# pierlj/ken-burns-effect

Hardware: AMD Instinct MI355X
Metric: novel_view_frames_per_sec_1024x1024 (higher is better)
Workload: dtype f32; 1 GPU; 1024x1024 KBE path, 1137109 pts (inpaint cloud), frame=shift+scatter+fill+u8+crop/resize; delivery=pinned_host, scatter_route=fused, frames_per_rank=1589, lanes=2, device_only_lanes=4, warmup_frames=3178, passes=1, handoff=sdma, ranks_seen=1

## Files before the change

### ken-burns-effect_amd/csrc/kbe_frame.hip

```cpp
#include <stdlib.h>
#include <string.h>

#include "kbe_cloud.h"
#include "kbe_handoff.h"
#include "kbe_tiles.h"

using namespace kbe;

namespace {

__global__ void k_scratch_init(uint32_t* zkeys, uint32_t* zkeys_b, size_t hw, int* tile_count, int n_tiles, int* hole_count)
{
    const size_t stride = (size_t) gridDim.x * blockDim.x, gtid = (size_t) blockIdx.x * blockDim.x + threadIdx.x;
    for (size_t i = gtid; i < hw; i += stride) { zkeys[i] = KBE_ZKEY_EMPTY; if (zkeys_b) zkeys_b[i] = KBE_ZKEY_EMPTY; }
    for (size_t i = gtid; i < (size_t) n_tiles; i += stride) { tile_count[i * CNT_STRIDE] = 0; tile_count[i * CNT_STRIDE + 1] = 0; }
    if (gtid < (size_t) HOLE_COUNT_INTS) hole_count[gtid] = 0;
}

__global__ void k_scratch_init_sets(char* base, size_t stride, size_t zkeys, size_t zkeys_b, size_t hw, size_t tile_count, int n_tiles, size_t hole_count)
{
    char* const set = base + (size_t) blockIdx.y * stride;
    uint32_t* const za = (uint32_t*) (set + zkeys), * const zb = (uint32_t*) (set + zkeys_b);
    const size_t step = (size_t) gridDim.x * blockDim.x, gtid = (size_t) blockIdx.x * blockDim.x + threadIdx.x;
    for (size_t i = gtid; i < hw; i += step) { za[i] = KBE_ZKEY_EMPTY; zb[i] = KBE_ZKEY_EMPTY; }
// ... 850 lines not shown
{
    KBE_REQUIRE(n_frames >= 0 && focals && shifts && stage && host_out && frame_size_ok(W, H) && batch >= -64 && (!packed || cloud_focal > 0.0),
                "kbe_render_video: bad arguments");
    KBE_REQUIRE((crop_w == 0 && crop_h == 0) || (crop_w > 0 && crop_h > 0 && crop_w <= W && crop_h <= H), "kbe_render_video: bad crop");
    KBE_REQUIRE(lanes >= 1 && lanes <= KBE_MAX_LANES && (lanes == 1 || lane_streams), "kbe_render_video: bad lanes");
    KBE_REQUIRE(near_depth >= 0.0 && near_depth < 1.0e30, "kbe_render_video: near_depth is a depth (0: unknown)");
    KBE_REQUIRE(scratch && ((uintptr_t) scratch & 15) == 0 && N >= 0 && (packed || (N <= (1 << 30) && (N == 0 || (points && image && depth)))),
                "kbe_render_video: bad scratch or cloud");
    const hipStream_t cs = (hipStream_t) stream;
    const size_t sb = (scratch_set_bytes(W, H, N) + 255) & ~(size_t) 255;
    const bool crop = crop_w > 0;
    const int wide_group = ((flags >> 5) & 15) + 1;
    const int group = batch <= 0 ? (wide_group > 1 ? wide_group : ((flags >> 1) & 3) + 1) : 1;
    KBE_REQUIRE(group <= (packed ? KBE_FRAME_JOBS : KBE_FILL_JOBS), "kbe_render_video: more frames per launch than the route's launches take");
    KBE_REQUIRE(!packed || N <= KBE_FUSED_MAX_POINTS, "kbe_render_video: the packed cloud's route takes up to 2^28 points (more: the plain cloud's route)");
    hipStream_t ls[KBE_MAX_LANES];
    for (int l = 0; l < lanes; l++) ls[l] = l == 0 ? cs : (hipStream_t) lane_streams[l];
    const StageLayout layout = stage_layout(W, H, lanes, batch, KBE_FRAME_JOBS);
    VideoHandoff handoff;
    if (int rc0 = handoff.open(HandoffIn{ stage, layout, host_out, batch, flags, lanes, ls, copy_stream ? (hipStream_t) copy_stream : cs })) return rc0;
    int rect[4] = { 0, 0, W - 1, H - 1 };
    if (crop) {
        const int x0 = (int) floor(W / 2.0 - (crop_w - 1) * 0.5) - 1, y0 = (int) floor(H / 2.0 - (crop_h - 1) * 0.5) - 1;
        rect[0] = x0 > 0 ? x0 : 0; rect[1] = y0 > 0 ? y0 : 0;
        rect[2] = x0 + crop_w + 2 < W - 1 ? x0 + crop_w + 2 : W - 1;
        rect[3] = y0 + crop_h + 2 < H - 1 ? y0 + crop_h + 2 : H - 1;
    }
    if (packed) {
        const Scratch sc0 = carve(scratch, W, H);
        hipLaunchKernelGGL(k_zero_counters, dim3(16, group * lanes), dim3(256), 0, cs, sc0.hole_count, sb, group * lanes, sc0.tile_count,
                           2 * align16(4 * (size_t) sc0.tiles_x * sc0.tiles_y * CNT_STRIDE) / sizeof(int));
        if (int rc0 = launched("kbe_render_video/counters")) return rc0;
    }
    const VideoPlan plan = plan_video(VideoPlanIn{ n_frames, lanes, group, batch, handoff.dest, layout.fin, (flags & KBE_VIDEO_FAST_RAMP) != 0, (flags & KBE_VIDEO_EVEN_GROUPS) != 0,
                                                   packed != nullptr, !(flags & KBE_VIDEO_NO_AHEAD) },
                                      [&](int n, int n_next) { return fused_can_place_ahead(N, W, H, n, n_next); });

    const int in_flight = plan.single ? lanes : lanes * group;
    const int fill_flags = in_flight >= KBE_FILL_BY_COUNT_MIN_LANES ? (KBE_STAGE_FILL_BY_COUNT | ((flags & KBE_VIDEO_FILL_DIST) ? KBE_STAGE_FILL_DIST : 0)) : 0;
    const int build = (flags & KBE_VIDEO_FUSED_LEAN) ? 1 : ((flags & KBE_VIDEO_FUSED_ROOMY) ? 2 : 0);
    const FillRect fill_rect = fill_rect_of(rect, W, H);
    auto fused_target_of = [&](const PlanFrame& f, uint8_t* frame, int turn) {
        return fused_target((char*) scratch + (size_t) f.set * sb, W, H, focals[f.frame], baseline, shifts + 3 * (size_t) f.frame, f.turn & 1, frame, turn);
    };
    auto render = [&](const PlanLaunch& a) {
        const hipStream_t s = ls[a.lane];
        const PlanFrame* const fr = &plan.frames[a.first];
        uint8_t* outs[KBE_FRAME_JOBS];
        uint8_t* raws[KBE_FRAME_JOBS];
        for (int j = 0; j < a.count; j++) {
            outs[j] = handoff.slot(fr[j]);
            raws[j] = crop ? stage + layout.raw(a.lane, j) : outs[j];
        }
        int rc = KBE_OK;
        if (!packed) {
            FrameJob jobs[KBE_FILL_JOBS];
            for (int j = 0; j < a.count; j++)
                jobs[j] = FrameJob{ focals[fr[j].frame], shifts + 3 * (size_t) fr[j].frame, (char*) scratch + (size_t) fr[j].set * sb, raws[j], nullptr, nullptr, nullptr, nullptr,
                                    fr[j].zbuf == PLAN_ZBUF_A ? KBE_STAGE_ZBUF_A : (fr[j].zbuf == PLAN_ZBUF_B ? KBE_STAGE_ZBUF_B : 0) };
            rc = render_jobs(points, image, depth, N, W, H, baseline, a.count, jobs, KBE_STAGE_PROJECT | KBE_STAGE_TILES | KBE_STAGE_FILL | fill_flags, crop ? rect : nullptr, raster_w, raster_n, s);
        } else if (plan.single) {
            const FusedTarget t = fused_target_of(fr[0], raws[0], -1);
            rc = render_fused(s, packed, N, cloud_focal, 1, &t, false, 0, nullptr, KBE_STAGE_TILES | KBE_STAGE_FILL | fill_flags, build, fill_rect, 0.0, "kbe_render_video");
        } else {
            FusedTarget ft[KBE_FRAME_JOBS], nt[KBE_FRAME_JOBS];
            for (int j = 0; j < a.count; j++) ft[j] = fused_target_of(fr[j], raws[j], fr[j].turn);
            const int n_next = a.next >= 0 ? plan.launches[a.next].count : 0;
            const PlanFrame* const next = n_next ? &plan.frames[plan.launches[a.next].first] : nullptr;
            for (int j = 0; j < n_next; j++) nt[j] = fused_target_of(next[j], nullptr, next[j].turn);
            rc = render_fused(s, packed, N, cloud_focal, a.count, ft, a.placed, n_next, nt, KBE_STAGE_TILES | KBE_STAGE_FILL | fill_flags, build, fill_rect, near_depth,
                              "kbe_render_video");
        }
        for (int j0 = 0; j0 < a.count && rc == KBE_OK && crop; j0 += KBE_FILL_JOBS)
            rc = crop_resize_group(a.count - j0 < KBE_FILL_JOBS ? a.count - j0 : KBE_FILL_JOBS, raws + j0, W, H, crop_w, crop_h, outs + j0, s);
        return rc;
    };

    int rc = handoff.start(plan);
    for (int u = 0; u < (int) plan.units.size() && rc == KBE_OK; u++) {
        const PlanUnit& un = plan.units[u];
        handoff.before(u, un);
        for (int a = un.launch0; a < un.launch1 && rc == KBE_OK; a++) rc = render(plan.launches[a]);
        if (rc == KBE_OK) rc = handoff.after(u, un, plan);
    }
    return handoff.finish(rc, plan);
}

}
```

### ken-burns-effect_amd/csrc/kbe_hip.hip

```cpp
#include <hip/hip_runtime.h>
#include <math.h>
#include <stdio.h>
#include <string.h>

#include "kbe.h"
#include "kbe_device.h"
#include "kbe_fill.h"
#include "kbe_host.h"

#pragma clang fp contract(off)

using namespace kbe;

thread_local char kbe::g_err[256] = "";

namespace {

__global__ void k_fill_u32(uint32_t* p, size_t n, uint32_t v)
{
    const size_t stride = (size_t) gridDim.x * blockDim.x;
    for (size_t i = (size_t) blockIdx.x * blockDim.x + threadIdx.x; i < n; i += stride) p[i] = v;
}

__global__ void k_zkeys_decode(const uint32_t* keys, size_t n, float* zee)
{
    const size_t stride = (size_t) gridDim.x * blockDim.x;
    for (size_t i = (size_t) blockIdx.x * blockDim.x + threadIdx.x; i < n; i += stride) zee[i] = zkey_decode(keys[i]);
}

__global__ void k_selftest_err(const float* __restrict__ z, size_t n, Camera cam, float* __restrict__ fast, float* __restrict__ exact)
{
    const size_t stride = (size_t) gridDim.x * blockDim.x;
    for (size_t i = (size_t) blockIdx.x * blockDim.x + threadIdx.x; i < n; i += stride) {
        fast[i] = project_err_fast(cam, z[i]);
        exact[i] = project_err(cam, z[i]);
    }
}

__global__ void k_selftest_division(const float* __restrict__ num, const float* __restrict__ den, size_t n, float* __restrict__ fast, float* __restrict__ ieee)
{
    const size_t stride = (size_t) gridDim.x * blockDim.x;
// ... 199 lines not shown

__device__ __forceinline__ void resize_coeff(int d, double scale, int src_n, bool horizontal, int& s0, int& s1, int& c0, int& c1)
{
    float f = (float) ((d + 0.5) * scale - 0.5);
    int s = (int) floorf(f);
    f -= (float) s;
    if (horizontal) {
        if (s < 0) { f = 0.f; s = 0; }
        if (s >= src_n - 1) { f = 0.f; s = src_n - 1; }
    }
    s0 = min(max(s, 0), src_n - 1);
    s1 = min(max(s + 1, 0), src_n - 1);
    c0 = cv_round((1.f - f) * 2048.f);
    c1 = cv_round(f * 2048.f);
}

__device__ __forceinline__ uint32_t mul_u24_v(uint32_t a, uint32_t b) { uint32_t r; asm("v_mul_u32_u24 %0, %1, %2" : "=v"(r) : "v"(a), "v"(b)); return r; }
__device__ __forceinline__ uint32_t mad_u24_v(uint32_t a, uint32_t b, uint32_t c) { uint32_t r; asm("v_mad_u32_u24 %0, %1, %2, %3" : "=v"(r) : "v"(a), "v"(b), "v"(c)); return r; }
__device__ __forceinline__ uint32_t mul_u24_s(uint32_t a, uint32_t b) { uint32_t r; asm("v_mul_u32_u24 %0, %1, %2" : "=v"(r) : "s"(a), "v"(b)); return r; }
__device__ __forceinline__ uint32_t mul_hi_u24_s(uint32_t a, uint32_t b) { uint32_t r; asm("v_mul_hi_u32_u24 %0, %1, %2" : "=v"(r) : "s"(a), "v"(b)); return r; }
__device__ __forceinline__ uint32_t mad_u24_s(uint32_t a, uint32_t b, uint32_t c) { uint32_t r; asm("v_mad_u32_u24 %0, %1, %2, %3" : "=v"(r) : "s"(a), "v"(b), "v"(c)); return r; }

#ifndef KBE_CROP_TH
#define KBE_CROP_TH 16
#endif
constexpr int CR_TW = 64, CR_TH = KBE_CROP_TH, CR_THREADS = 256, CR_WAVES = CR_THREADS / 64;
constexpr int CR_ROWS_PER_WAVE = CR_TH / CR_WAVES;
constexpr int CR_PROWS = CR_TH + 2, CR_PCOLS = CR_TW + 2;
constexpr int CR_PBYTES = CR_PCOLS * 3, CR_PSTRIDE = (CR_PBYTES + 3) / 4 + 1;
constexpr int CR_RROWS = CR_PROWS + 1, CR_RDW = ((CR_PCOLS + 1) * 3 + 3 + 3) / 4 + 1;
constexpr int CR_STAGE = (CR_RROWS + CR_WAVES - 1) / CR_WAVES;
static_assert(CR_TH % CR_WAVES == 0 && CR_RDW <= 64 && CR_PBYTES <= CR_THREADS && CR_TW + CR_TH <= CR_THREADS && CR_PROWS + 1 <= CR_THREADS, "crop tile geometry");

__device__ __forceinline__ void crop_resize_body(const uint8_t* __restrict__ img, int W, int H, int cw, int ch_, double scale_x, double scale_y, uint8_t* __restrict__ out)
{
    __shared__ uint32_t s_raw[CR_RROWS][CR_RDW];
    __shared__ uint32_t s_patch[CR_PROWS][CR_PSTRIDE];
    __shared__ __attribute__((aligned(16))) uint32_t s_out[CR_TH][CR_TW * 3 / 4];
    __shared__ int s_cx[4][CR_TW], s_cy[4][CR_TH];
    __shared__ int s_ro[CR_PROWS + 1];
    const int tid = threadIdx.x;
    const int bx = blockIdx.x * CR_TW, by = blockIdx.y * CR_TH;
    const float cx = (float) W / 2.0f - (float) (cw - 1) * 0.5f, cy = (float) H / 2.0f - (float) (ch_ - 1) * 0.5f;
    const int ipx = (int) floorf(cx), ipy = (int) floorf(cy);
    const float fa = cx - (float) ipx, fb = cy - (float) ipy;
    const int a11 = cv_round((1.f - fa) * (1.f - fb) * 65536.f), a12 = cv_round(fa * (1.f - fb) * 65536.f);
    const int a21 = cv_round((1.f - fa) * fb * 65536.f), a22 = cv_round(fa * fb * 65536.f);
    const bool whole = (a12 | a21 | a22) == 0;
    if (tid < CR_TW + CR_TH) {
        const bool col = tid < CR_TW;
        const int k = col ? tid : tid - CR_TW;
        int s0, s1, c0, c1;
        if (col) resize_coeff(min(bx + k, W - 1), scale_x, cw, true, s0, s1, c0, c1);
        else resize_coeff(min(by + k, H - 1), scale_y, ch_, false, s0, s1, c0, c1);
        int* t = col ? &s_cx[0][k] : &s_cy[0][k];
        const int stride = col ? CR_TW : CR_TH;
        t[0] = s0; t[stride] = s1; t[2 * stride] = c0; t[3 * stride] = c1;
    }
    __syncthreads();
    const int px_lo = s_cx[0][0], px_hi = s_cx[1][CR_TW - 1], py_lo = s_cy[0][0], py_hi = s_cy[1][CR_TH - 1];
    const int n_pc3 = (px_hi - px_lo + 1) * 3, n_pr = py_hi - py_lo + 1;
    const int rx0 = min(max(ipx + px_lo, 0), W - 1), rx1 = min(max(ipx + px_hi + 1, 0), W - 1);
    const int ry0 = min(max(ipy + py_lo, 0), H - 1), ry1 = min(max(ipy + py_hi + 1, 0), H - 1);
    const int n_rows = ry1 - ry0 + 1;
    const size_t frame_bytes = (size_t) W * H * 3;
    const int wv = __builtin_amdgcn_readfirstlane(tid >> 6), ln = tid & 63;
    uint32_t stage[CR_STAGE];
#pragma unroll
    for (int k = 0; k < CR_STAGE; k++) {
        const int r = wv + CR_WAVES * k;
        stage[k] = 0;
        if (r < n_rows) {
            const size_t b0 = ((size_t) (ry0 + r) * W + rx0) * 3, b1 = ((size_t) (ry0 + r) * W + rx1) * 3 + 3;
            const size_t a0 = b0 & ~(size_t) 3;
            const int n_dw = (int) ((b1 - a0 + 3) >> 2);
            const uint8_t* row = img + a0;
            if (a0 + 4 * (size_t) n_dw <= frame_bytes) {
                if (ln < n_dw) stage[k] = ((const uint32_t*) row)[ln];
            } else if (ln < n_dw) {
                for (int t = 0; t < 4; t++) if (a0 + 4 * (size_t) ln + t < frame_bytes) stage[k] |= (uint32_t) row[4 * ln + t] << (8 * t);
            }
        }
    }
#pragma unroll
    for (int k = 0; k < CR_STAGE; k++) {
        const int r = wv + CR_WAVES * k;
        if (r < CR_RROWS && ln < CR_RDW) s_raw[r][ln] = stage[k];
    }
    if (tid <= CR_PROWS) {
        const int y = min(max(ipy + py_lo + tid, 0), H - 1);
        s_ro[tid] = min(y - ry0, CR_RROWS - 1) * (int) sizeof(s_raw[0]) + (int) ((((uint32_t) y * (uint32_t) W + (uint32_t) rx0) * 3u) & 3u);
    }
    __syncthreads();
    const uint8_t* raw = (const uint8_t*) s_raw;
    uint8_t* patch = (uint8_t*) s_patch;
    if (!whole) {
        if (tid < n_pc3) {
            const int pc = tid / 3, c = tid - pc * 3;
            const int x0 = (min(max(ipx + px_lo + pc, 0), W - 1) - rx0) * 3 + c, x1 = (min(max(ipx + px_lo + pc + 1, 0), W - 1) - rx0) * 3 + c;
            int o = s_ro[0];
            int t0 = raw[o + x0], t1 = raw[o + x1];
            for (int pr = 0; pr < n_pr; pr++) {
                o = s_ro[pr + 1];
                const int u0 = raw[o + x0], u1 = raw[o + x1];
                const uint32_t t = mad_u24_s((uint32_t) a22, (uint32_t) u1, mad_u24_s((uint32_t) a21, (uint32_t) u0, mad_u24_s((uint32_t) a12, (uint32_t) t1, mad_u24_s((uint32_t) a11, (uint32_t) t0, 1u << 15))));
                patch[pr * (int) sizeof(s_patch[0]) + tid] = (uint8_t) (t >> 16);
                t0 = u0; t1 = u1;
            }
        }
        __syncthreads();
    }
    const int col = tid & (CR_TW - 1);
    const uint8_t* const src = whole ? raw : (const uint8_t*) patch;
    int sx, sx1;
    if (whole) {
        sx = (min(max(ipx + s_cx[0][col], 0), W - 1) - rx0) * 3;
        sx1 = (min(max(ipx + s_cx[1][col], 0), W - 1) - rx0) * 3;
    } else {
        sx = (s_cx[0][col] - px_lo) * 3;
        sx1 = (s_cx[1][col] - px_lo) * 3;
    }
    const int ax0 = s_cx[2][col], ax1 = s_cx[3][col];
    auto row_offset = [&](int pr) -> int {
        return whole ? s_ro[pr] : pr * (int) sizeof(s_patch[0]);
    };
    auto horizontal = [&](int pr, int (&h)[3]) {
        const int o = row_offset(pr);
#pragma unroll
        for (int c = 0; c < 3; c++) h[c] = (int) (mad_u24_v(src[o + sx1 + c], (uint32_t) ax1, mul_u24_v(src[o + sx + c], (uint32_t) ax0)) & ~15u);
    };
    int ka = -1, kb = -1;
    int ha[3] = { 0, 0, 0 }, hb[3] = { 0, 0, 0 };
    uint8_t px[CR_ROWS_PER_WAVE][3];
#pragma unroll
    for (int m = 0; m < CR_ROWS_PER_WAVE; m++) {
        const int row = wv * CR_ROWS_PER_WAVE + m;
        const int y0 = __builtin_amdgcn_readfirstlane(s_cy[0][row] - py_lo), y1 = __builtin_amdgcn_readfirstlane(s_cy[1][row] - py_lo);
        const int by0 = __builtin_amdgcn_readfirstlane(s_cy[2][row]), by1 = __builtin_amdgcn_readfirstlane(s_cy[3][row]);
        if (ka != y0) {
            if (kb == y0) {
#pragma unroll
                for (int c = 0; c < 3; c++) ha[c] = hb[c];
            } else horizontal(y0, ha);
            ka = y0;
        }
        if (y1 == y0) {
#pragma unroll
            for (int c = 0; c < 3; c++) hb[c] = ha[c];
            kb = y0;
        } else if (kb != y1) { horizontal(y1, hb); kb = y1; }
#pragma unroll
        for (int c = 0; c < 3; c++) {
            const uint32_t v = (mul_hi_u24_s((uint32_t) by0 << 12, (uint32_t) ha[c]) + mul_hi_u24_s((uint32_t) by1 << 12, (uint32_t) hb[c]) + 2u) >> 2;
            px[m][c] = (uint8_t) v;
        }
        uint8_t* so = (uint8_t*) s_out[row] + col * 3;
        so[0] = px[m][0]; so[1] = px[m][1]; so[2] = px[m][2];
    }
    __syncthreads();
    if ((W & 15) == 0 && bx + CR_TW <= W && ((uintptr_t) out & 15) == 0) {
        constexpr int Q = CR_TW * 3 / 16;
        static_assert((CR_TW * 3) % 16 == 0 && sizeof(s_out[0]) % 16 == 0, "16-byte row stores");
        for (int i = tid; i < CR_TH * Q; i += CR_THREADS) {
            const int r = i / Q, k = i - r * Q;
            if (by + r < H) ((uint4*) (out + ((size_t) (by + r) * W + bx) * 3))[k] = ((const uint4*) s_out[r])[k];
        }
    } else if ((W & 3) == 0 && bx + CR_TW <= W && ((uintptr_t) out & 3) == 0) {
        constexpr int DW = CR_TW * 3 / 4;
        for (int i = tid; i < CR_TH * DW; i += CR_THREADS) {
            const int r = i / DW, k = i - r * DW;
            if (by + r < H) ((uint32_t*) (out + ((size_t) (by + r) * W + bx) * 3))[k] = s_out[r][k];
        }
    } else {
#pragma unroll
        for (int m = 0; m < CR_ROWS_PER_WAVE; m++) {
            const int dx = bx + col, dy = by + wv * CR_ROWS_PER_WAVE + m;
            if (dx < W && dy < H) {
                const size_t o = ((size_t) dy * W + dx) * 3;
                out[o] = px[m][0]; out[o + 1] = px[m][1]; out[o + 2] = px[m][2];
            }
        }
    }
}

__global__ void __launch_bounds__(CR_THREADS) k_crop_resize_u8(const uint8_t* __restrict__ img, int W, int H, int cw, int ch_, double scale_x, double scale_y,
                                                               uint8_t* __restrict__ out)
{
    crop_resize_body(img, W, H, cw, ch_, scale_x, scale_y, out);
}

struct CropJobs { const uint8_t* img[4]; uint8_t* out[4]; };
__global__ void __launch_bounds__(CR_THREADS) k_crop_resize_u8_group(CropJobs jobs, int W, int H, int cw, int ch_, double scale_x, double scale_y)
{
    crop_resize_body(jobs.img[blockIdx.z], W, H, cw, ch_, scale_x, scale_y, jobs.out[blockIdx.z]);
}


__device__ __forceinline__ float linspace_centered(int n, int i)
{
    const float start = (float) ((-0.5 * n) + 0.5), end = (float) ((0.5 * n) - 0.5);
    if (n == 1) return start;
    const float step = (end - start) / (float) (n - 1);
    return (i < n / 2) ? start + step * (float) i : end - step * (float) (n - 1 - i);
}

__global__ void __launch_bounds__(kBlock) k_depth_to_points(const float* __restrict__ depth, const float* __restrict__ valid,
                                                            int W, int H, float inv_focal, float* __restrict__ points)
{
    const int b = blockIdx.y;
    const int HW = W * H;
    const int i = blockIdx.x * blockDim.x + threadIdx.x;
    if (i >= HW) return;
    const int y = i / W, x = i - y * W;
    float d = depth[(size_t) b * HW + i];
    if (valid) d = d * valid[(size_t) b * HW + i];
    const float u = linspace_centered(W, x) * inv_focal;
    const float v = linspace_centered(H, y) * inv_focal;
    float* P = points + (size_t) b * 3 * HW;
    P[i] = d * u;
    P[(size_t) HW + i] = d * v;
    P[(size_t) 2 * HW + i] = d;
}

__global__ void __launch_bounds__(kBlock) k_shift_points(const float* __restrict__ points, int N, Camera cam,
                                                         float* __restrict__ out)
{
    const int b = blockIdx.y;
// ... 316 lines not shown
    int rc;
    if ((rc = kbe_zkeys_clear(zkeys, (size_t) B * H * W, stream))) return rc;
    const hipError_t e = hipMemsetAsync(acc, 0, sizeof(float) * (size_t) B * (C + 1) * H * W, (hipStream_t) stream);
    if (e != hipSuccess) return fail(KBE_E_LAUNCH, "hipMemsetAsync(acc)", e);
    if ((rc = kbe_zsplat(points, B, N, W, H, focal, baseline, nullptr, zkeys, nullptr, stream))) return rc;
    if ((rc = kbe_degrid(zkeys, nullptr, B, W, H, zee, stream))) return rc;
    if ((rc = kbe_accumulate(points, data, B, N, C, zee, W, H, focal, baseline, nullptr, acc, stream))) return rc;
    return kbe_normalize(acc, B, C, W, H, render, existing, stream);
}

int kbe_fill_disocclusion(const float* input, const float* depth, int B, int C, int W, int H, float* output,
                          kbe_stream_t stream)
{
    KBE_REQUIRE(input && depth && output && B > 0 && C > 0 && W > 0 && H > 0, "kbe_fill_disocclusion: bad arguments");
    static const FillDirs dirs = make_fill_dirs();
    hipLaunchKernelGGL(k_fill, dim3(blocks_for((size_t) W * H), B), dim3(kBlock), 0, (hipStream_t) stream, input, depth, C,
                       W, H, dirs, output);
    return launched("kbe_fill_disocclusion");
}

int kbe_frame_u8(const float* render_chw, int W, int H, uint8_t* frame_hwc, kbe_stream_t stream)
{
    KBE_REQUIRE(render_chw && frame_hwc && W > 0 && H > 0, "kbe_frame_u8: bad arguments");
    hipLaunchKernelGGL(k_frame_u8, dim3(blocks_for((size_t) W * H)), dim3(kBlock), 0, (hipStream_t) stream, render_chw,
                       W * H, frame_hwc);
    return launched("kbe_frame_u8");
}

int kbe_crop_resize_u8(const uint8_t* frame_hwc, int W, int H, int crop_w, int crop_h, uint8_t* out_hwc,
                       kbe_stream_t stream)
{
    KBE_REQUIRE(frame_hwc && out_hwc && W > 0 && H > 0 && crop_w > 0 && crop_h > 0 && crop_w <= W && crop_h <= H,
                "kbe_crop_resize_u8: bad arguments");
    hipLaunchKernelGGL(k_crop_resize_u8, dim3((W + CR_TW - 1) / CR_TW, (H + CR_TH - 1) / CR_TH), dim3(CR_THREADS), 0,
                       (hipStream_t) stream, frame_hwc, W, H, crop_w, crop_h, (double) crop_w / W, (double) crop_h / H, out_hwc);
    return launched("kbe_crop_resize_u8");
}

}

namespace kbe {
int crop_resize_group(int n, const uint8_t* const* frames, int W, int H, int crop_w, int crop_h, uint8_t* const* outs, hipStream_t stream)
{
    if (n == 1) return kbe_crop_resize_u8(frames[0], W, H, crop_w, crop_h, outs[0], (kbe_stream_t) stream);
    CropJobs jobs;
    for (int k = 0; k < 4; k++) { jobs.img[k] = frames[k < n ? k : 0]; jobs.out[k] = outs[k < n ? k : 0]; }
    hipLaunchKernelGGL(k_crop_resize_u8_group, dim3((W + CR_TW - 1) / CR_TW, (H + CR_TH - 1) / CR_TH, n), dim3(CR_THREADS), 0, stream, jobs, W, H, crop_w, crop_h, (double) crop_w / W, (double) crop_h / H);
    return launched("kbe_crop_resize_u8 (group)");
}
}

extern "C" {

int kbe_depth_to_points(const float* depth, const float* valid, int B, int W, int H, double focal, float* points,
                        kbe_stream_t stream)
{
    KBE_REQUIRE(depth && points && B > 0 && W > 0 && H > 0, "kbe_depth_to_points: bad arguments");
    const float inv = (float) (1.0 / focal);
    hipLaunchKernelGGL(k_depth_to_points, dim3(blocks_for((size_t) W * H), B), dim3(kBlock), 0, (hipStream_t) stream, depth,
                       valid, W, H, inv, points);
    return launched("kbe_depth_to_points");
}

int kbe_shift_points(const float* points, int B, int N, const float* shift3, float* out, kbe_stream_t stream)
{
    KBE_REQUIRE(shift3 && B > 0 && N >= 0, "kbe_shift_points: bad arguments");
    if (N == 0) return KBE_OK;
    KBE_REQUIRE(points && out, "kbe_shift_points: points/out is NULL");
    const Camera cam = make_camera(1, 1, 1.0, 1.0, shift3);
    hipLaunchKernelGGL(k_shift_points, dim3(blocks_for(N), B), dim3(kBlock), 0, (hipStream_t) stream, points, N, cam, out);
    return launched("kbe_shift_points");
}

int kbe_spatial_filter(const float* in, int planes, int W, int H, int kind, float* out, kbe_stream_t stream)
{
    KBE_REQUIRE(in && out && planes > 0 && W > 0 && H > 0, "kbe_spatial_filter: bad arguments");
    const dim3 grid(blocks_for((size_t) W * H), planes);
    const hipStream_t s = (hipStream_t) stream;
    if (kind == 0) {
        hipLaunchKernelGGL(k_laplacian<false>, grid, dim3(kBlock), 0, s, in, (const float*) nullptr, W, H, 0.0f, out);
// ... 60 lines not shown
```

### ken-burns-effect_amd/csrc/kbe_tiles.h

```cpp
#pragma once
#include <hip/hip_runtime.h>
#include <math.h>
#include <stddef.h>
#include <stdint.h>
#include <type_traits>

#include "kbe.h"
#include "kbe_device.h"
#include "kbe_fill.h"
#include "kbe_host.h"
#include "kbe_cloud.h"

#pragma clang fp contract(off)

namespace kbe {

#ifndef KBE_TILE_W
#define KBE_TILE_W 32
#endif
#ifndef KBE_TILE_H
#define KBE_TILE_H 16
#endif
#ifndef KBE_TILE_THREADS
#define KBE_TILE_THREADS 256
#endif
#ifndef KBE_TILE_CAP
#define KBE_TILE_CAP 736
#endif
#ifndef KBE_BUCKET_FACTOR
#define KBE_BUCKET_FACTOR 12
#endif
constexpr int TW = KBE_TILE_W, TH = KBE_TILE_H;
constexpr int KW = TW + 2, KH = TH + 2;
constexpr int BW = TW + 1, BH = TH + 1;
constexpr int TILE_THREADS = KBE_TILE_THREADS;
constexpr int PIX_PER_THREAD = TW * TH / TILE_THREADS;
constexpr int REC_CAP = KBE_TILE_CAP;
constexpr int BUCKET_CAP = KBE_BUCKET_FACTOR * TW * TH;
#ifndef KBE_BUCKET_PAD
#define KBE_BUCKET_PAD 272
#endif
constexpr int BUCKET_STRIDE = BUCKET_CAP + KBE_BUCKET_PAD;
#ifndef KBE_CAND_CAP
#define KBE_CAND_CAP (2048 * 16 / KBE_CLOUD_SUB)
#endif
constexpr int CNT_STRIDE = 32;
static_assert(TW * TH % TILE_THREADS == 0 && TILE_THREADS % 64 == 0 && REC_CAP >= TILE_THREADS && TW % 32 == 0, "tile geometry");

struct Scratch {
    uint32_t* zkeys;
    uint32_t* zkeys_b;
    uint8_t* dist;
    float2* strips;
    uint8_t* dist_blocks;
    int* tile_count;
    int* hole_count;
    int4* bbox;
    uint32_t* coarse;
    int* holes;
    float* depth;
    uint32_t* mask;
    int* cand;
    float4* buckets;
    int tiles_x, tiles_y;
};

inline size_t align16(size_t v) { return (v + 15) & ~(size_t) 15; }

inline Scratch carve(void* base, int W, int H)
{
    char* p = (char*) base;
    const size_t hw = (size_t) W * H;
    Scratch s;
    s.tiles_x = (W + TW - 1) / TW;
    s.tiles_y = (H + TH - 1) / TH;
    const size_t n_tiles = (size_t) s.tiles_x * s.tiles_y;
    s.zkeys = (uint32_t*) p;      p += align16(4 * hw);
    s.tile_count = (int*) p;      p += 2 * align16(4 * n_tiles * CNT_STRIDE);
    s.hole_count = (int*) p;      p += 32;
    s.bbox = (int4*) p;           p += align16(16 * n_tiles);
    s.coarse = (uint32_t*) p;     p += align16(4 * n_tiles);
    s.holes = (int*) p;           p += align16(4 * hw);
    s.depth = (float*) p;         p += align16(4 * hw);
    s.mask = (uint32_t*) p;       p += align16(4 * (size_t) H * ((W + 31) / 32));
    s.zkeys_b = (uint32_t*) p;    p += align16(4 * hw);
    s.dist = (uint8_t*) p;        p += align16(hw);
    s.strips = (float2*) p;       p += align16(8 * 16 * (size_t) (W + H + 8));
    s.dist_blocks = (uint8_t*) p; p += align16(n_tiles * (TW / 8) * (TH / 8));
    s.cand = (int*) p;            p += 2 * align16(4 * n_tiles * KBE_CAND_CAP);
    s.buckets = (float4*) p;
    return s;
}

inline size_t scratch_bytes(int W, int H)
{
    const size_t hw = (size_t) W * H;
    const size_t n_tiles = (size_t) ((W + TW - 1) / TW) * ((H + TH - 1) / TH);
    return align16(4 * hw) + 2 * align16(4 * n_tiles * CNT_STRIDE) + 32 + align16(16 * n_tiles) + align16(4 * n_tiles) + align16(4 * hw) + align16(4 * hw) +
           align16(4 * (size_t) H * ((W + 31) / 32)) + align16(4 * hw) + align16(hw) + align16(8 * 16 * (size_t) (W + H + 8)) + align16(n_tiles * (TW / 8) * (TH / 8)) + 2 * align16(4 * n_tiles * KBE_CAND_CAP) + n_tiles * BUCKET_STRIDE * sizeof(float4);
}


size_t fused_place_bytes(int N);
inline size_t scratch_set_bytes(int W, int H, int N) { return align16(scratch_bytes(W, H)) + (N >= 0 ? 2 * align16(fused_place_bytes(N)) : 0); }
inline void* scratch_place(void* base, int W, int H) { return (char*) base + align16(scratch_bytes(W, H)); }
inline int* bank_tile_count(const Scratch& s, int bank) { return (int*) ((char*) s.tile_count + (size_t) bank * align16(4 * (size_t) s.tiles_x * s.tiles_y * CNT_STRIDE)); }
inline int* bank_cand(const Scratch& s, int bank) { return (int*) ((char*) s.cand + (size_t) bank * align16(4 * (size_t) s.tiles_x * s.tiles_y * KBE_CAND_CAP)); }
inline void* bank_place(void* place, int N, int bank) { return (char*) place + (size_t) bank * align16(fused_place_bytes(N)); }
constexpr int HOLE_COUNT_INTS = 8;

struct FillRect { int x0, y0, x1, y1; };

#ifndef KBE_FILL_BY_COUNT_MIN_LANES
#define KBE_FILL_BY_COUNT_MIN_LANES 2
#endif

constexpr int KBE_FILL_JOBS = 4;
#ifndef KBE_FRAME_JOBS_MAX
#define KBE_FRAME_JOBS_MAX 12
#endif
constexpr int KBE_FUSED_MAX_POINTS = 1 << 28;
constexpr int KBE_FRAME_JOBS = KBE_FRAME_JOBS_MAX;
struct FillTarget {
    Scratch sc;
    const int* hole_count;
    uint8_t* frame_u8;
    float* render_f32;
    int reset_scatter_scratch;
    int* next_hole_count;
};
struct FillJob {
    const int* holes; const int* hole_count; const float* depth; const uint32_t* mask; uint8_t* frame; float* render;
    uint32_t* zkeys; int* tile_count; const int4* bbox; const uint32_t* coarse; uint8_t* dist; float2* strips; uint8_t* dist_blocks;
    int reset_scatter_scratch; int* next_hole_count;
};
struct FillJobs { FillJob j[KBE_FILL_JOBS]; };
void launch_fill(hipStream_t s, int n_jobs, const FillTarget* targets, int W, int H, int stages, const FillDirs& dirs, const FillRect& rect, int n_tiles);
int crop_resize_group(int n, const uint8_t* const* frames, int W, int H, int crop_w, int crop_h, uint8_t* const* outs, hipStream_t stream);
struct FusedTarget {
    Camera cam;
    Scratch sc;
    void* place;
    int parity;
    uint8_t* frame_u8;
    float* render_f32; float* existing_f32; float* zee_f32; float* zee_pre_f32;
    int turn;
};
void launch_frames_fused(hipStream_t s, int n, const void* packed, int N, double cloud_focal, const FusedTarget* targets, bool placed = false, int n_next = 0,
                         const FusedTarget* next = nullptr, int build = 0, double near_depth = 0.0);
inline int fused_build_of_stages(int stages) { return (stages & 1024) ? 1 : ((stages & 2048) ? 2 : 0); }
bool fused_can_place_ahead(int N, int W, int H, int n, int n_next);

__device__ __forceinline__ int xcd_tile(int b, int n)
{
    const int xcd = b & 7, j = b >> 3, q = n >> 3, r = n & 7;
    return (xcd < r ? xcd * (q + 1) : r * (q + 1) + (xcd - r) * q) + j;
}
__device__ __forceinline__ int xcd_tile_rot(int b, int n, int job)
{
    if (n & 7) return xcd_tile(b, n);
    const int stride = gridDim.y >= 8 ? 1 : 8 / (int) gridDim.y;
    return (((b + job * stride) & 7) * (n >> 3)) + (b >> 3);
}

typedef float f2 __attribute__((ext_vector_type(2)));
typedef float f4 __attribute__((ext_vector_type(4)));
struct PixAcc { f2 rg, bd; float w; };

template <int CAP> struct TileLdsT {
    static constexpr int kCap = CAP;
    static constexpr int kDummy = CAP;
// ... 239 lines not shown
```

### ken-burns-effect_amd/csrc/kbe_video_plan.h

```cpp
#pragma once
#include <stddef.h>
#include <vector>

namespace kbe {

enum class VideoDest {
    HBM,
    PER_FRAME,
    GROUPS,
    RING,
};
enum { PLAN_ZBUF_ALONE = 0, PLAN_ZBUF_A = 1, PLAN_ZBUF_B = 2 };

struct StageLayout {
    size_t fb;
    int fin;
    size_t raw_per_lane, finished, ring, ctl, total;
    size_t raw(int lane, int j) const { return (raw_per_lane * lane + j) * fb; }
};
inline StageLayout stage_layout(int W, int H, int lanes, int batch, int raw_per_lane)
{
    const size_t fb = (size_t) W * H * 3, fin = batch < -2 ? -batch : 2;
    const size_t finished = (size_t) raw_per_lane * lanes * fb, ring = finished + fin * lanes * fb;
    const size_t ctl = (ring + 2 * (size_t) (batch > 0 ? batch : 0) * fb + 255) & ~(size_t) 255;
    return StageLayout{ fb, (int) fin, (size_t) raw_per_lane, finished, ring, ctl, ctl + 256 };
}

struct VideoPlanIn {
    int n_frames, lanes, group, batch;
    VideoDest dest;
    int fin;
    bool fast_ramp, even_groups;
    bool fused;
    bool ahead;
};
struct PlanFrame {
    int frame;
    int set;
    int turn;
    int zbuf;
    int slot;
};
struct PlanLaunch {
    int lane, first, count;
    bool placed;
    int next;
};
struct PlanUnit {
    int lane;
    int first, count;
    int launch0, launch1;
};
struct VideoPlan {
    bool single;
    std::vector<PlanUnit> units;
    std::vector<PlanLaunch> launches;
    std::vector<PlanFrame> frames;
};
// ... 71 lines not shown
```

Before: 17750 frames/s.

## Precompute crop-resize coefficient table once per video and specialize kernel on whole-pixel crop

```diff
diff --git a/ken-burns-effect_amd/csrc/kbe_frame.hip b/ken-burns-effect_amd/csrc/kbe_frame.hip
--- a/ken-burns-effect_amd/csrc/kbe_frame.hip
+++ b/ken-burns-effect_amd/csrc/kbe_frame.hip
@@ -906,6 +906,9 @@
                            2 * align16(4 * (size_t) sc0.tiles_x * sc0.tiles_y * CNT_STRIDE) / sizeof(int));
         if (int rc0 = launched("kbe_render_video/counters")) return rc0;
     }
+    int* const crop_table = carve(scratch, W, H).crop_table;
+    if (crop)
+        if (int rc0 = crop_table_build(W, H, crop_w, crop_h, crop_table, cs)) return rc0;
     const VideoPlan plan = plan_video(VideoPlanIn{ n_frames, lanes, group, batch, handoff.dest, layout.fin, (flags & KBE_VIDEO_FAST_RAMP) != 0, (flags & KBE_VIDEO_EVEN_GROUPS) != 0,
                                                    packed != nullptr, !(flags & KBE_VIDEO_NO_AHEAD) },
                                       [&](int n, int n_next) { return fused_can_place_ahead(N, W, H, n, n_next); });
@@ -946,7 +949,7 @@
                               "kbe_render_video");
         }
         for (int j0 = 0; j0 < a.count && rc == KBE_OK && crop; j0 += KBE_FILL_JOBS)
-            rc = crop_resize_group(a.count - j0 < KBE_FILL_JOBS ? a.count - j0 : KBE_FILL_JOBS, raws + j0, W, H, crop_w, crop_h, outs + j0, s);
+            rc = crop_resize_group(a.count - j0 < KBE_FILL_JOBS ? a.count - j0 : KBE_FILL_JOBS, raws + j0, W, H, crop_w, crop_h, outs + j0, crop_table, s);
         return rc;
     };
 
diff --git a/ken-burns-effect_amd/csrc/kbe_hip.hip b/ken-burns-effect_amd/csrc/kbe_hip.hip
--- a/ken-burns-effect_amd/csrc/kbe_hip.hip
+++ b/ken-burns-effect_amd/csrc/kbe_hip.hip
@@ -2,11 +2,16 @@
 #include <math.h>
 #include <stdio.h>
 #include <string.h>
+#include <type_traits>
+#ifdef KBE_DEBUG
+#include <assert.h>
+#endif
 
 #include "kbe.h"
 #include "kbe_device.h"
 #include "kbe_fill.h"
 #include "kbe_host.h"
+#include "kbe_video_plan.h"
 
 #pragma clang fp contract(off)
 
@@ -272,53 +277,143 @@
 constexpr int CR_STAGE = (CR_RROWS + CR_WAVES - 1) / CR_WAVES;
 static_assert(CR_TH % CR_WAVES == 0 && CR_RDW <= 64 && CR_PBYTES <= CR_THREADS && CR_TW + CR_TH <= CR_THREADS && CR_PROWS + 1 <= CR_THREADS, "crop tile geometry");
 
-__device__ __forceinline__ void crop_resize_body(const uint8_t* __restrict__ img, int W, int H, int cw, int ch_, double scale_x, double scale_y, uint8_t* __restrict__ out)
-{
-    __shared__ uint32_t s_raw[CR_RROWS][CR_RDW];
-    __shared__ uint32_t s_patch[CR_PROWS][CR_PSTRIDE];
-    __shared__ __attribute__((aligned(16))) uint32_t s_out[CR_TH][CR_TW * 3 / 4];
-    __shared__ int s_cx[4][CR_TW], s_cy[4][CR_TH];
-    __shared__ int s_ro[CR_PROWS + 1];
-    const int tid = threadIdx.x;
-    const int bx = blockIdx.x * CR_TW, by = blockIdx.y * CR_TH;
+template <class RowOffset>
+__device__ __forceinline__ void crop_resize_rows(const uint8_t* src, int sx, int sx1, int ax0, int ax1, const int4 (&cye)[CR_ROWS_PER_WAVE], int py_lo, int wv, int col,
+                                                 RowOffset row_offset, uint32_t (&s_out)[CR_TH][CR_TW * 3 / 4])
+{
+    auto horizontal = [&](int pr, int (&h)[3]) {
+        const int o = row_offset(pr);
+#pragma unroll
+        for (int c = 0; c < 3; c++) h[c] = (int) (mad_u24_v(src[o + sx1 + c], (uint32_t) ax1, mul_u24_v(src[o + sx + c], (uint32_t) ax0)) & ~15u);
+    };
+    int ka = -1, kb = -1;
+    int ha[3] = { 0, 0, 0 }, hb[3] = { 0, 0, 0 };
+#pragma unroll
+    for (int m = 0; m < CR_ROWS_PER_WAVE; m++) {
+        const int row = wv * CR_ROWS_PER_WAVE + m;
+        const int y0 = cye[m].x - py_lo, y1 = cye[m].y - py_lo;
+        const int by0 = cye[m].z, by1 = cye[m].w;
+        if (ka != y0) {
+            if (kb == y0) {
+#pragma unroll
+                for (int c = 0; c < 3; c++) ha[c] = hb[c];
+            } else horizontal(y0, ha);
+            ka = y0;
+        }
+        if (y1 == y0) {
+#pragma unroll
+            for (int c = 0; c < 3; c++) hb[c] = ha[c];
+            kb = y0;
+        } else if (kb != y1) { horizontal(y1, hb); kb = y1; }
+        uint8_t* so = (uint8_t*) s_out[row] + col * 3;
+#pragma unroll
+        for (int c = 0; c < 3; c++) {
+            const uint32_t v = (mul_hi_u24_s((uint32_t) by0 << 12, (uint32_t) ha[c]) + mul_hi_u24_s((uint32_t) by1 << 12, (uint32_t) hb[c]) + 2u) >> 2;
+            so[c] = (uint8_t) v;
+        }
+    }
+}
+
+struct CropHeader { int ipx, ipy, a11, a12, a21, a22, whole, pad; };
+static_assert(sizeof(CropHeader) == crop_table_layout(1, 1).cols && crop_table_layout(3, 1).rows == sizeof(CropHeader) + 3 * sizeof(int4), "the table's header: 8 dwords, then the columns, then the rows (kbe_video_plan.h: crop_table_layout)");
+__host__ __device__ __forceinline__ CropHeader crop_header(int W, int H, int cw, int ch_)
+{
     const float cx = (float) W / 2.0f - (float) (cw - 1) * 0.5f, cy = (float) H / 2.0f - (float) (ch_ - 1) * 0.5f;
     const int ipx = (int) floorf(cx), ipy = (int) floorf(cy);
     const float fa = cx - (float) ipx, fb = cy - (float) ipy;
-    const int a11 = cv_round((1.f - fa) * (1.f - fb) * 65536.f), a12 = cv_round(fa * (1.f - fb) * 65536.f);
-    const int a21 = cv_round((1.f - fa) * fb * 65536.f), a22 = cv_round(fa * fb * 65536.f);
-    const bool whole = (a12 | a21 | a22) == 0;
-    if (tid < CR_TW + CR_TH) {
-        const bool col = tid < CR_TW;
-        const int k = col ? tid : tid - CR_TW;
-        int s0, s1, c0, c1;
-        if (col) resize_coeff(min(bx + k, W - 1), scale_x, cw, true, s0, s1, c0, c1);
-        else resize_coeff(min(by + k, H - 1), scale_y, ch_, false, s0, s1, c0, c1);
-        int* t = col ? &s_cx[0][k] : &s_cy[0][k];
-        const int stride = col ? CR_TW : CR_TH;
-        t[0] = s0; t[stride] = s1; t[2 * stride] = c0; t[3 * stride] = c1;
-    }
-    __syncthreads();
-    const int px_lo = s_cx[0][0], px_hi = s_cx[1][CR_TW - 1], py_lo = s_cy[0][0], py_hi = s_cy[1][CR_TH - 1];
+    const int a11 = (int) rintf((1.f - fa) * (1.f - fb) * 65536.f), a12 = (int) rintf(fa * (1.f - fb) * 65536.f);
+    const int a21 = (int) rintf((1.f - fa) * fb * 65536.f), a22 = (int) rintf(fa * fb * 65536.f);
+    return CropHeader{ ipx, ipy, a11, a12, a21, a22, (a12 | a21 | a22) == 0, 0 };
+}
+
+__global__ void __launch_bounds__(kBlock) k_crop_table(int W, int H, int cw, int ch_, double scale_x, double scale_y, int* __restrict__ table)
+{
+    const int i = blockIdx.x * blockDim.x + threadIdx.x;
+    if (i == 0) *(CropHeader*) table = crop_header(W, H, cw, ch_);
+    if (i >= W + H) return;
+    int s0, s1, c0, c1;
+    if (i < W) resize_coeff(i, scale_x, cw, true, s0, s1, c0, c1);
+    else resize_coeff(i - W, scale_y, ch_, false, s0, s1, c0, c1);
+    ((int4*) (table + sizeof(CropHeader) / sizeof(int)))[i] = make_int4(s0, s1, c0, c1);
+}
+
+template <bool WHOLE, bool TABLE>
+__device__ __forceinline__ void crop_resize_body(const uint8_t* __restrict__ img, int W, int H, int cw, int ch_, double scale_x, double scale_y,
+                                                 const int* __restrict__ table, uint8_t* __restrict__ out)
+{
+    using offs_t = std::conditional_t<TABLE, uint32_t, size_t>;
+    __shared__ uint32_t s_raw[CR_RROWS][CR_RDW];
+    __shared__ __attribute__((aligned(16))) uint32_t s_out[CR_TH][CR_TW * 3 / 4];
+    const int tid = threadIdx.x;
+    const int bx = blockIdx.x * CR_TW, by = blockIdx.y * CR_TH;
+    const int wv = __builtin_amdgcn_readfirstlane(tid >> 6), ln = tid & 63;
+    const int col = tid & (CR_TW - 1);
+    auto uni = [](int v) { return __builtin_amdgcn_readfirstlane(v); };
+    CropHeader hd;
+    int4 cxe, cye[CR_ROWS_PER_WAVE];
+    int px_lo, px_hi, py_lo, py_hi;
+    if constexpr (TABLE) {
+        const CropHeader* const th = (const CropHeader*) table;
+        const int4* const cols = (const int4*) (table + sizeof(CropHeader) / sizeof(int));
+        const int4* const rows = cols + W;
+        hd.ipx = uni(th->ipx); hd.ipy = uni(th->ipy);
+        if constexpr (!WHOLE) { hd.a11 = uni(th->a11); hd.a12 = uni(th->a12); hd.a21 = uni(th->a21); hd.a22 = uni(th->a22); }
+#ifdef KBE_DEBUG
+        assert((th->whole != 0) == WHOLE);
+#endif
+        cxe = cols[min(bx + col, W - 1)];
+#pragma unroll
+        for (int m = 0; m < CR_ROWS_PER_WAVE; m++) {
+            const int4 e = rows[min(by + wv * CR_ROWS_PER_WAVE + m, H - 1)];
+            cye[m] = make_int4(uni(e.x), uni(e.y), uni(e.z), uni(e.w));
+        }
+        px_lo = uni(cols[min(bx, W - 1)].x); px_hi = uni(cols[min(bx + CR_TW - 1, W - 1)].y);
+        py_lo = uni(rows[min(by, H - 1)].x); py_hi = uni(rows[min(by + CR_TH - 1, H - 1)].y);
+    } else {
+        __shared__ int s_cx[4][CR_TW], s_cy[4][CR_TH];
+        hd = crop_header(W, H, cw, ch_);
+#ifdef KBE_DEBUG
+        assert((hd.whole != 0) == WHOLE);
+#endif
+        if (tid < CR_TW + CR_TH) {
+            const bool is_col = tid < CR_TW;
+            const int k = is_col ? tid : tid - CR_TW;
+            int s0, s1, c0, c1;
+            if (is_col) resize_coeff(min(bx + k, W - 1), scale_x, cw, true, s0, s1, c0, c1);
+            else resize_coeff(min(by + k, H - 1), scale_y, ch_, false, s0, s1, c0, c1);
+            int* t = is_col ? &s_cx[0][k] : &s_cy[0][k];
+            const int stride = is_col ? CR_TW : CR_TH;
+            t[0] = s0; t[stride] = s1; t[2 * stride] = c0; t[3 * stride] = c1;
+        }
+        __syncthreads();
+        cxe = make_int4(s_cx[0][col], s_cx[1][col], s_cx[2][col], s_cx[3][col]);
+#pragma unroll
+        for (int m = 0; m < CR_ROWS_PER_WAVE; m++) {
+            const int row = wv * CR_ROWS_PER_WAVE + m;
+            cye[m] = make_int4(uni(s_cy[0][row]), uni(s_cy[1][row]), uni(s_cy[2][row]), uni(s_cy[3][row]));
+        }
+        px_lo = uni(s_cx[0][0]); px_hi = uni(s_cx[1][CR_TW - 1]); py_lo = uni(s_cy[0][0]); py_hi = uni(s_cy[1][CR_TH - 1]);
+    }
+    const int ipx = hd.ipx, ipy = hd.ipy;
     const int n_pc3 = (px_hi - px_lo + 1) * 3, n_pr = py_hi - py_lo + 1;
     const int rx0 = min(max(ipx + px_lo, 0), W - 1), rx1 = min(max(ipx + px_hi + 1, 0), W - 1);
     const int ry0 = min(max(ipy + py_lo, 0), H - 1), ry1 = min(max(ipy + py_hi + 1, 0), H - 1);
     const int n_rows = ry1 - ry0 + 1;
-    const size_t frame_bytes = (size_t) W * H * 3;
-    const int wv = __builtin_amdgcn_readfirstlane(tid >> 6), ln = tid & 63;
+    const offs_t frame_bytes = (offs_t) W * H * 3;
     uint32_t stage[CR_STAGE];
 #pragma unroll
     for (int k = 0; k < CR_STAGE; k++) {
         const int r = wv + CR_WAVES * k;
         stage[k] = 0;
         if (r < n_rows) {
-            const size_t b0 = ((size_t) (ry0 + r) * W + rx0) * 3, b1 = ((size_t) (ry0 + r) * W + rx1) * 3 + 3;
-            const size_t a0 = b0 & ~(size_t) 3;
+            const offs_t b0 = ((offs_t) (ry0 + r) * W + rx0) * 3, b1 = ((offs_t) (ry0 + r) * W + rx1) * 3 + 3;
+            const offs_t a0 = b0 & ~(offs_t) 3;
             const int n_dw = (int) ((b1 - a0 + 3) >> 2);
             const uint8_t* row = img + a0;
-            if (a0 + 4 * (size_t) n_dw <= frame_bytes) {
+            if (a0 + 4 * (offs_t) n_dw <= frame_bytes) {
                 if (ln < n_dw) stage[k] = ((const uint32_t*) row)[ln];
             } else if (ln < n_dw) {
-                for (int t = 0; t < 4; t++) if (a0 + 4 * (size_t) ln + t < frame_bytes) stage[k] |= (uint32_t) row[4 * ln + t] << (8 * t);
+                for (int t = 0; t < 4; t++) if (a0 + 4 * (offs_t) ln + t < frame_bytes) stage[k] |= (uint32_t) row[4 * ln + t] << (8 * t);
             }
         }
     }
@@ -327,14 +422,21 @@
         const int r = wv + CR_WAVES * k;
         if (r < CR_RROWS && ln < CR_RDW) s_raw[r][ln] = stage[k];
     }
-    if (tid <= CR_PROWS) {
-        const int y = min(max(ipy + py_lo + tid, 0), H - 1);
-        s_ro[tid] = min(y - ry0, CR_RROWS - 1) * (int) sizeof(s_raw[0]) + (int) ((((uint32_t) y * (uint32_t) W + (uint32_t) rx0) * 3u) & 3u);
-    }
-    __syncthreads();
+    auto raw_row_offset = [&](int pr) -> int {
+        const int y = min(max(ipy + py_lo + pr, 0), H - 1);
+        return min(y - ry0, CR_RROWS - 1) * (int) sizeof(s_raw[0]) + (int) ((((uint32_t) y * (uint32_t) W + (uint32_t) rx0) * 3u) & 3u);
+    };
     const uint8_t* raw = (const uint8_t*) s_raw;
-    uint8_t* patch = (uint8_t*) s_patch;
-    if (!whole) {
+    if constexpr (WHOLE) {
+        __syncthreads();
+        const int sx = (min(max(ipx + cxe.x, 0), W - 1) - rx0) * 3, sx1 = (min(max(ipx + cxe.y, 0), W - 1) - rx0) * 3;
+        crop_resize_rows(raw, sx, sx1, cxe.z, cxe.w, cye, py_lo, wv, col, raw_row_offset, s_out);
+    } else {
+        __shared__ uint32_t s_patch[CR_PROWS][CR_PSTRIDE];
+        __shared__ int s_ro[CR_PROWS + 1];
+        if (tid <= CR_PROWS) s_ro[tid] = raw_row_offset(tid);
+        __syncthreads();
+        uint8_t* patch = (uint8_t*) s_patch;
         if (tid < n_pc3) {
             const int pc = tid / 3, c = tid - pc * 3;
             const int x0 = (min(max(ipx + px_lo + pc, 0), W - 1) - rx0) * 3 + c, x1 = (min(max(ipx + px_lo + pc + 1, 0), W - 1) - rx0) * 3 + c;
@@ -343,59 +445,13 @@
             for (int pr = 0; pr < n_pr; pr++) {
                 o = s_ro[pr + 1];
                 const int u0 = raw[o + x0], u1 = raw[o + x1];
-                const uint32_t t = mad_u24_s((uint32_t) a22, (uint32_t) u1, mad_u24_s((uint32_t) a21, (uint32_t) u0, mad_u24_s((uint32_t) a12, (uint32_t) t1, mad_u24_s((uint32_t) a11, (uint32_t) t0, 1u << 15))));
+                const uint32_t t = mad_u24_s((uint32_t) hd.a22, (uint32_t) u1, mad_u24_s((uint32_t) hd.a21, (uint32_t) u0, mad_u24_s((uint32_t) hd.a12, (uint32_t) t1, mad_u24_s((uint32_t) hd.a11, (uint32_t) t0, 1u << 15))));
                 patch[pr * (int) sizeof(s_patch[0]) + tid] = (uint8_t) (t >> 16);
                 t0 = u0; t1 = u1;
             }
         }
         __syncthreads();
-    }
-    const int col = tid & (CR_TW - 1);
-    const uint8_t* const src = whole ? raw : (const uint8_t*) patch;
-    int sx, sx1;
-    if (whole) {
-        sx = (min(max(ipx + s_cx[0][col], 0), W - 1) - rx0) * 3;
-        sx1 = (min(max(ipx + s_cx[1][col], 0), W - 1) - rx0) * 3;
-    } else {
-        sx = (s_cx[0][col] - px_lo) * 3;
-        sx1 = (s_cx[1][col] - px_lo) * 3;
-    }
-    const int ax0 = s_cx[2][col], ax1 = s_cx[3][col];
-    auto row_offset = [&](int pr) -> int {
-        return whole ? s_ro[pr] : pr * (int) sizeof(s_patch[0]);
-    };
-    auto horizontal = [&](int pr, int (&h)[3]) {
-        const int o = row_offset(pr);
-#pragma unroll
-        for (int c = 0; c < 3; c++) h[c] = (int) (mad_u24_v(src[o + sx1 + c], (uint32_t) ax1, mul_u24_v(src[o + sx + c], (uint32_t) ax0)) & ~15u);
-    };
-    int ka = -1, kb = -1;
-    int ha[3] = { 0, 0, 0 }, hb[3] = { 0, 0, 0 };
-    uint8_t px[CR_ROWS_PER_WAVE][3];
-#pragma unroll
-    for (int m = 0; m < CR_ROWS_PER_WAVE; m++) {
-        const int row = wv * CR_ROWS_PER_WAVE + m;
-        const int y0 = __builtin_amdgcn_readfirstlane(s_cy[0][row] - py_lo), y1 = __builtin_amdgcn_readfirstlane(s_cy[1][row] - py_lo);
-        const int by0 = __builtin_amdgcn_readfirstlane(s_cy[2][row]), by1 = __builtin_amdgcn_readfirstlane(s_cy[3][row]);
-        if (ka != y0) {
-            if (kb == y0) {
-#pragma unroll
-                for (int c = 0; c < 3; c++) ha[c] = hb[c];
-            } else horizontal(y0, ha);
-            ka = y0;
-        }
-        if (y1 == y0) {
-#pragma unroll
-            for (int c = 0; c < 3; c++) hb[c] = ha[c];
-            kb = y0;
-        } else if (kb != y1) { horizontal(y1, hb); kb = y1; }
-#pragma unroll
-        for (int c = 0; c < 3; c++) {
-            const uint32_t v = (mul_hi_u24_s((uint32_t) by0 << 12, (uint32_t) ha[c]) + mul_hi_u24_s((uint32_t) by1 << 12, (uint32_t) hb[c]) + 2u) >> 2;
-            px[m][c] = (uint8_t) v;
-        }
-        uint8_t* so = (uint8_t*) s_out[row] + col * 3;
-        so[0] = px[m][0]; so[1] = px[m][1]; so[2] = px[m][2];
+        crop_resize_rows(patch, (cxe.x - px_lo) * 3, (cxe.y - px_lo) * 3, cxe.z, cxe.w, cye, py_lo, wv, col, [](int pr) -> int { return pr * (int) sizeof(s_patch[0]); }, s_out);
     }
     __syncthreads();
     if ((W & 15) == 0 && bx + CR_TW <= W && ((uintptr_t) out & 15) == 0) {
@@ -403,36 +459,40 @@
         static_assert((CR_TW * 3) % 16 == 0 && sizeof(s_out[0]) % 16 == 0, "16-byte row stores");
         for (int i = tid; i < CR_TH * Q; i += CR_THREADS) {
             const int r = i / Q, k = i - r * Q;
-            if (by + r < H) ((uint4*) (out + ((size_t) (by + r) * W + bx) * 3))[k] = ((const uint4*) s_out[r])[k];
+            if (by + r < H) ((uint4*) (out + ((offs_t) (by + r) * W + bx) * 3))[k] = ((const uint4*) s_out[r])[k];
         }
     } else if ((W & 3) == 0 && bx + CR_TW <= W && ((uintptr_t) out & 3) == 0) {
         constexpr int DW = CR_TW * 3 / 4;
         for (int i = tid; i < CR_TH * DW; i += CR_THREADS) {
             const int r = i / DW, k = i - r * DW;
-            if (by + r < H) ((uint32_t*) (out + ((size_t) (by + r) * W + bx) * 3))[k] = s_out[r][k];
+            if (by + r < H) ((uint32_t*) (out + ((offs_t) (by + r) * W + bx) * 3))[k] = s_out[r][k];
         }
     } else {
 #pragma unroll
         for (int m = 0; m < CR_ROWS_PER_WAVE; m++) {
-            const int dx = bx + col, dy = by + wv * CR_ROWS_PER_WAVE + m;
+            const int row = wv * CR_ROWS_PER_WAVE + m;
+            const int dx = bx + col, dy = by + row;
             if (dx < W && dy < H) {
-                const size_t o = ((size_t) dy * W + dx) * 3;
-                out[o] = px[m][0]; out[o + 1] = px[m][1]; out[o + 2] = px[m][2];
+                const offs_t o = ((offs_t) dy * W + dx) * 3;
+                const uint8_t* so = (const uint8_t*) s_out[row] + col * 3;
+                out[o] = so[0]; out[o + 1] = so[1]; out[o + 2] = so[2];
             }
         }
     }
 }
 
+template <bool WHOLE>
 __global__ void __launch_bounds__(CR_THREADS) k_crop_resize_u8(const uint8_t* __restrict__ img, int W, int H, int cw, int ch_, double scale_x, double scale_y,
                                                                uint8_t* __restrict__ out)
 {
-    crop_resize_body(img, W, H, cw, ch_, scale_x, scale_y, out);
+    crop_resize_body<WHOLE, false>(img, W, H, cw, ch_, scale_x, scale_y, nullptr, out);
 }
 
 struct CropJobs { const uint8_t* img[4]; uint8_t* out[4]; };
-__global__ void __launch_bounds__(CR_THREADS) k_crop_resize_u8_group(CropJobs jobs, int W, int H, int cw, int ch_, double scale_x, double scale_y)
-{
-    crop_resize_body(jobs.img[blockIdx.z], W, H, cw, ch_, scale_x, scale_y, jobs.out[blockIdx.z]);
+template <bool WHOLE>
+__global__ void __launch_bounds__(CR_THREADS) k_crop_resize_u8_group(CropJobs jobs, int W, int H, int cw, int ch_, const int* __restrict__ table)
+{
+    crop_resize_body<WHOLE, true>(jobs.img[blockIdx.z], W, H, cw, ch_, 0.0, 0.0, table, jobs.out[blockIdx.z]);
 }
 
 
@@ -815,7 +875,8 @@
 {
     KBE_REQUIRE(frame_hwc && out_hwc && W > 0 && H > 0 && crop_w > 0 && crop_h > 0 && crop_w <= W && crop_h <= H,
                 "kbe_crop_resize_u8: bad arguments");
-    hipLaunchKernelGGL(k_crop_resize_u8, dim3((W + CR_TW - 1) / CR_TW, (H + CR_TH - 1) / CR_TH), dim3(CR_THREADS), 0,
+    const auto kernel = crop_header(W, H, crop_w, crop_h).whole ? k_crop_resize_u8<true> : k_crop_resize_u8<false>;
+    hipLaunchKernelGGL(kernel, dim3((W + CR_TW - 1) / CR_TW, (H + CR_TH - 1) / CR_TH), dim3(CR_THREADS), 0,
                        (hipStream_t) stream, frame_hwc, W, H, crop_w, crop_h, (double) crop_w / W, (double) crop_h / H, out_hwc);
     return launched("kbe_crop_resize_u8");
 }
@@ -823,12 +884,20 @@
 }
 
 namespace kbe {
-int crop_resize_group(int n, const uint8_t* const* frames, int W, int H, int crop_w, int crop_h, uint8_t* const* outs, hipStream_t stream)
-{
-    if (n == 1) return kbe_crop_resize_u8(frames[0], W, H, crop_w, crop_h, outs[0], (kbe_stream_t) stream);
+int crop_table_build(int W, int H, int crop_w, int crop_h, int* table, hipStream_t stream)
+{
+    KBE_REQUIRE(table && ((uintptr_t) table & 15) == 0 && W > 0 && H > 0 && crop_w > 0 && crop_h > 0 && crop_w <= W && crop_h <= H, "crop_table_build: bad arguments");
+    hipLaunchKernelGGL(k_crop_table, dim3(blocks_for((size_t) W + H)), dim3(kBlock), 0, stream, W, H, crop_w, crop_h, (double) crop_w / W, (double) crop_h / H, table);
+    return launched("kbe_crop_resize_u8 (table)");
+}
+
+int crop_resize_group(int n, const uint8_t* const* frames, int W, int H, int crop_w, int crop_h, uint8_t* const* outs, const int* table, hipStream_t stream)
+{
+    KBE_REQUIRE(n >= 1 && n <= 4 && table && (size_t) W * H <= (1u << 30), "crop_resize_group: bad arguments");
     CropJobs jobs;
     for (int k = 0; k < 4; k++) { jobs.img[k] = frames[k < n ? k : 0]; jobs.out[k] = outs[k < n ? k : 0]; }
-    hipLaunchKernelGGL(k_crop_resize_u8_group, dim3((W + CR_TW - 1) / CR_TW, (H + CR_TH - 1) / CR_TH, n), dim3(CR_THREADS), 0, stream, jobs, W, H, crop_w, crop_h, (double) crop_w / W, (double) crop_h / H);
+    const auto kernel = crop_header(W, H, crop_w, crop_h).whole ? k_crop_resize_u8_group<true> : k_crop_resize_u8_group<false>;
+    hipLaunchKernelGGL(kernel, dim3((W + CR_TW - 1) / CR_TW, (H + CR_TH - 1) / CR_TH, n), dim3(CR_THREADS), 0, stream, jobs, W, H, crop_w, crop_h, table);
     return launched("kbe_crop_resize_u8 (group)");
 }
 }
diff --git a/ken-burns-effect_amd/csrc/kbe_tiles.h b/ken-burns-effect_amd/csrc/kbe_tiles.h
--- a/ken-burns-effect_amd/csrc/kbe_tiles.h
+++ b/ken-burns-effect_amd/csrc/kbe_tiles.h
@@ -10,6 +10,7 @@
 #include "kbe_fill.h"
 #include "kbe_host.h"
 #include "kbe_cloud.h"
+#include "kbe_video_plan.h"
 
 #pragma clang fp contract(off)
 
@@ -62,6 +63,7 @@
     uint32_t* mask;
     int* cand;
     float4* buckets;
+    int* crop_table;
     int tiles_x, tiles_y;
 };
 
@@ -88,7 +90,8 @@
     s.strips = (float2*) p;       p += align16(8 * 16 * (size_t) (W + H + 8));
     s.dist_blocks = (uint8_t*) p; p += align16(n_tiles * (TW / 8) * (TH / 8));
     s.cand = (int*) p;            p += 2 * align16(4 * n_tiles * KBE_CAND_CAP);
-    s.buckets = (float4*) p;
+    s.buckets = (float4*) p;      p += n_tiles * BUCKET_STRIDE * sizeof(float4);
+    s.crop_table = (int*) p;
     return s;
 }
 
@@ -97,7 +100,8 @@
     const size_t hw = (size_t) W * H;
     const size_t n_tiles = (size_t) ((W + TW - 1) / TW) * ((H + TH - 1) / TH);
     return align16(4 * hw) + 2 * align16(4 * n_tiles * CNT_STRIDE) + 32 + align16(16 * n_tiles) + align16(4 * n_tiles) + align16(4 * hw) + align16(4 * hw) +
-           align16(4 * (size_t) H * ((W + 31) / 32)) + align16(4 * hw) + align16(hw) + align16(8 * 16 * (size_t) (W + H + 8)) + align16(n_tiles * (TW / 8) * (TH / 8)) + 2 * align16(4 * n_tiles * KBE_CAND_CAP) + n_tiles * BUCKET_STRIDE * sizeof(float4);
+           align16(4 * (size_t) H * ((W + 31) / 32)) + align16(4 * hw) + align16(hw) + align16(8 * 16 * (size_t) (W + H + 8)) + align16(n_tiles * (TW / 8) * (TH / 8)) + 2 * align16(4 * n_tiles * KBE_CAND_CAP) + n_tiles * BUCKET_STRIDE * sizeof(float4) +
+           crop_table_layout(W, H).total;
 }
 
 
@@ -136,7 +140,8 @@
 };
 struct FillJobs { FillJob j[KBE_FILL_JOBS]; };
 void launch_fill(hipStream_t s, int n_jobs, const FillTarget* targets, int W, int H, int stages, const FillDirs& dirs, const FillRect& rect, int n_tiles);
-int crop_resize_group(int n, const uint8_t* const* frames, int W, int H, int crop_w, int crop_h, uint8_t* const* outs, hipStream_t stream);
+int crop_table_build(int W, int H, int crop_w, int crop_h, int* table, hipStream_t stream);
+int crop_resize_group(int n, const uint8_t* const* frames, int W, int H, int crop_w, int crop_h, uint8_t* const* outs, const int* table, hipStream_t stream);
 struct FusedTarget {
     Camera cam;
     Scratch sc;
diff --git a/ken-burns-effect_amd/csrc/kbe_video_plan.h b/ken-burns-effect_amd/csrc/kbe_video_plan.h
--- a/ken-burns-effect_amd/csrc/kbe_video_plan.h
+++ b/ken-burns-effect_amd/csrc/kbe_video_plan.h
@@ -24,6 +24,13 @@
     const size_t finished = (size_t) raw_per_lane * lanes * fb, ring = finished + fin * lanes * fb;
     const size_t ctl = (ring + 2 * (size_t) (batch > 0 ? batch : 0) * fb + 255) & ~(size_t) 255;
     return StageLayout{ fb, (int) fin, (size_t) raw_per_lane, finished, ring, ctl, ctl + 256 };
+}
+
+struct CropTableLayout { size_t header, cols, rows, total; };
+constexpr CropTableLayout crop_table_layout(int W, int H)
+{
+    const size_t header = 0, cols = header + 8 * sizeof(int), rows = cols + 16 * (size_t) W;
+    return CropTableLayout{ header, cols, rows, rows + 16 * (size_t) H };
 }
 
 struct VideoPlanIn {
```

Result: no change. 17630 frames/s (median of 2 runs) (-0.7%).
